# narayanan2004/GraphMat

Measured on AMD Instinct MI355X. Metric: GTEPS (edges/s) per iter + achieved HBM GB/s, PageRank RMAT-26, higher is better.
Workload: dtype f32

## Files before the change

### include/graphmat/kernels.hpp

```cpp
#pragma once
#include <hip/hip_runtime.h>
#include <stdint.h>
#include <string.h>

#include <type_traits>

#include "../graphmat_hip.h"

namespace GraphMat {

enum reduce_kind {
  REDUCE_AUTO = -1,
  REDUCE_ORDERED = 0,
  REDUCE_COMMUTATIVE = 1,
  REDUCE_LAST = 2,
  REDUCE_F32_ADD = 3
};

template <class P>
struct program_traits {
  static constexpr reduce_kind reduce = REDUCE_AUTO;
};

template <class P>
// ... 951 lines not shown
      const int v = stream_load(&A.colidx[k]);
      c[r] = pos < lr ? v : -1;
    }
  };
  auto msgs = [&]() {
#pragma unroll
    for (int r = 0; r < G; r++) {
      const int cc = c[r];
      const unsigned rel = (unsigned)(cc - hot.base);
      bool in_lds = rel < (unsigned)hot.nhot;
      unsigned slot = rel;
#ifdef GRAPHMAT_ABLATION
      if (cc >= 0 && abl_cold(cc, hot.cold_from, hot.base)) { in_lds = true; slot = (unsigned)cc & 4095u; }
      if (dbg & DBG_SKIP_GATHER) { in_lds = true; slot = 0; }
#endif
      const T mh = hot.s_hot[in_lds ? slot : 0u];
      const T* __restrict__ ga = (in_lds || cc < 0) ? xdummy : x + cc;
      const T mg = *ga;
      m[r] = in_lds ? mh : mg;
    }
  };
  cols(0);
  msgs();
  if (nsteps > 1) cols(1);
  for (int step = 0; step < nsteps; step++) {
#pragma unroll
    for (int r = 0; r < G; r++) {
      U term;
      const int kraw = __builtin_amdgcn_readlane(mt.e0, r) + step * 64 + lane;
      const int k = (int64_t)kraw < A.nnz ? kraw : (int)(A.nnz - 1);
      p.P::process_message(m[r], edge_at<E>(A.vals, k), no_vp, term);
      s_t[r][lane] = term;
    }
    __builtin_amdgcn_wave_barrier();
    if (step + 1 < nsteps) {
      msgs();
      if (step + 2 < nsteps) cols(step + 2);
    }
    if (lane < G && !(dbg & DBG_SKIP_FOLD)) {
      int n = mt.len - step * 64;
      n = n > 64 ? 64 : n;
      const U* t = s_t[lane];
      if (n == 64) {
        int k = 0;
        if (!has) { acc = t[0]; has = true; k = 1; }
        for (; k < 64; k++) { U v = t[k]; p.P::reduce_function(acc, v); }
      } else if (n > 0) {
        int k = 0;
        if (!has) { acc = t[0]; has = true; k = 1; }
        U nx[4];
        if (k + 4 <= n) {
#pragma unroll
          for (int u = 0; u < 4; u++) nx[u] = t[k + u];
        }
        while (k + 4 <= n) {
          U cur[4];
#pragma unroll
          for (int u = 0; u < 4; u++) cur[u] = nx[u];
          k += 4;
          if (k + 4 <= n) {
#pragma unroll
            for (int u = 0; u < 4; u++) nx[u] = t[k + u];
          }
#pragma unroll
          for (int u = 0; u < 4; u++) p.P::reduce_function(acc, cur[u]);
        }
        for (; k < n; k++) { U v = t[k]; p.P::reduce_function(acc, v); }
      }
    }
    __builtin_amdgcn_wave_barrier();
  }
  if (lane < G && mt.row >= 0 && has) {
    y[mt.row] = acc;
    if (!(accumulate & ACC_STATIC_BITS)) atomicOr(&ybits[mt.row >> 5], 1u << (mt.row & 31));
  }
}
template <class P, class T>
__device__ __forceinline__ bool w16_dense_ok(const gm_csr_t& A, const uint32_t* xbits, const uint32_t* want, const HotSet<T>& hot) {
  return xbits == nullptr && want == nullptr && !program_row_filter<P>::enabled && hot.NS == 1 && A.nnz < ((int64_t)1 << 31) && A.nnz > 0;
}

template <class P, class T, class U, class V, class E>
__global__ void __launch_bounds__(kWave16Block)
k_spmv_wave16(ProgArg<P> pa, gm_csr_t A, const int32_t* __restrict__ rows, int nlist, const T* __restrict__ x,
              const uint32_t* __restrict__ xbits, const V* __restrict__ vp, U* __restrict__ y,
              uint32_t* __restrict__ ybits, int accumulate GM_DBG_PARAM, const uint32_t* __restrict__ want) {
  static_assert(sizeof(U) == 4 || sizeof(U) == 8, "LDS tile of 4- or 8-byte products");
  constexpr int G = kWaveRows;
  constexpr int kStride = 64 + 16 / (int)sizeof(U);
  __shared__ __attribute__((aligned(16))) U s_t[kWave16Block / 64][G][kStride];
  __shared__ unsigned long long s_mask[kWave16Block / 64][G];
  constexpr int kHot = sizeof(T) == 4 ? kHotEntries : 1;
  __shared__ T s_hot[kHot];
  const HotSet<T> hot = hot_load<T, kHot, kWave16Block>(A, x, s_hot);
  __syncthreads();
  const P& p = *reinterpret_cast<const P*>(pa.b);
  const int wv = threadIdx.x >> 6, lane = threadIdx.x & 63;
  const int first = (blockIdx.x * (kWave16Block / 64) + wv) * G;
  if (first >= nlist) return;
  wave16_group<P, T, U, V, E, kStride>(p, A, rows, nlist, first, lane, x, xbits, vp, y, ybits, accumulate GM_DBG_PASS, want, hot, s_t[wv], s_mask[wv]);
}

template <class P, class T, class U, class V, class E, int BLOCK, int HOT>
__global__ void __launch_bounds__(BLOCK)
k_spmv_wave16p(ProgArg<P> pa, gm_csr_t A, const int32_t* __restrict__ rows, int nlist, const T* __restrict__ x,
               const uint32_t* __restrict__ xbits, const V* __restrict__ vp, U* __restrict__ y,
               uint32_t* __restrict__ ybits, int accumulate GM_DBG_PARAM, const uint32_t* __restrict__ want) {
  static_assert(sizeof(U) == 4 || sizeof(U) == 8, "LDS tile of 4- or 8-byte products");
  static_assert(sizeof(T) == 4, "4-byte messages");
  constexpr int G = kWaveRows;
  constexpr int kStride = 64 + 16 / (int)sizeof(U);
  __shared__ __attribute__((aligned(16))) U s_t[BLOCK / 64][G][kStride];
  __shared__ unsigned long long s_mask[BLOCK / 64][G];
  __shared__ T s_hot[HOT];
#ifdef GRAPHMAT_ABLATION
  const unsigned long long abl_t0 = wall_clock64();
#endif
  const HotSet<T> hot = hot_load<T, HOT, BLOCK>(A, x, s_hot);
  __syncthreads();
  const P& p = *reinterpret_cast<const P*>(pa.b);
  const int wv = threadIdx.x >> 6, lane = threadIdx.x & 63;
  const int ngroups = (nlist + G - 1) / G;
  const int nwaves = gridDim.x * (BLOCK / 64);
#ifdef GRAPHMAT_ABLATION
  const unsigned long long abl_t1 = wall_clock64();
  struct AblStamp {
    unsigned long long t0, t1;
    int w, lane;
    __device__ ~AblStamp() {
      if (lane == 0 && w < 8192) {
        g_abl_wave_times[0][w][0] = t0; g_abl_wave_times[0][w][1] = t1; g_abl_wave_times[0][w][2] = wall_clock64();
      }
    }
  } abl_stamp{abl_t0, abl_t1, (int)(blockIdx.x * (BLOCK / 64) + wv), lane};
#endif
  if (w16_dense_ok<P, T>(A, xbits, want, hot) && !(dbg & DBG_PLAIN_WAVE16)) {
    int g = wv * gridDim.x + blockIdx.x;
    int row_n = w16_row(rows, nlist, g + nwaves < ngroups ? (g + nwaves) * G : -1, lane);
    W16Meta<U> cur = w16_meta<U>(A, w16_row(rows, nlist, g < ngroups ? g * G : -1, lane), y, ybits, accumulate);
    while (g < ngroups) {
      const int gn = g + nwaves;
      const int row_nn = w16_row(rows, nlist, gn + nwaves < ngroups ? (gn + nwaves) * G : -1, lane);
      const W16Meta<U> nxt = w16_meta<U>(A, row_n, y, ybits, accumulate);
      wave16_dense<P, T, U, V, E, kStride>(p, A, cur, lane, x, y, ybits, accumulate GM_DBG_PASS, hot, s_t[wv]);
      cur = nxt;
      row_n = row_nn;
      g = gn;
    }
    return;
  }
  for (int g = wv * gridDim.x + blockIdx.x; g < ngroups; g += nwaves)
    wave16_group<P, T, U, V, E, kStride>(p, A, rows, nlist, g * G, lane, x, xbits, vp, y, ybits, accumulate GM_DBG_PASS, want, hot, s_t[wv], s_mask[wv]);
}

template <class P, class T, class U, class V, class E, int BLOCK, int HOT>
__global__ void __launch_bounds__(BLOCK)
k_spmv_rowwave(ProgArg<P> pa, gm_csr_t A, const T* __restrict__ x, U* __restrict__ y, uint32_t* __restrict__ ybits, int accumulate) {
  static_assert(sizeof(T) == 4, "4-byte messages");
  constexpr int W = BLOCK / 64;
  constexpr int CH = 512, PER = CH / 64;
  constexpr int kPadw = CH + CH / 32;
  __shared__ T s_hot[HOT > 0 ? HOT : 1];
  __shared__ T s_msg[W][kPadw];
#define GM_WSLOT(k) ((k) + ((k) >> 5))
#ifdef GRAPHMAT_ABLATION
  const unsigned long long abl_t0 = wall_clock64();
#endif
  const HotSet<T> hot = hot_load<T, HOT, BLOCK>(A, x, s_hot);
  __syncthreads();
  const P& p = *reinterpret_cast<const P*>(pa.b);
  const int wv = threadIdx.x >> 6, lane = threadIdx.x & 63;
#ifdef GRAPHMAT_ABLATION
  const unsigned long long abl_t1 = wall_clock64();
  struct AblStamp {
    unsigned long long t0, t1;
    int w, lane;
    __device__ ~AblStamp() {
      if (lane == 0 && w < 8192) {
        g_abl_wave_times[1][w][0] = t0; g_abl_wave_times[1][w][1] = t1; g_abl_wave_times[1][w][2] = wall_clock64();
      }
    }
  } abl_stamp{abl_t0, abl_t1, (int)(blockIdx.x * (BLOCK / 64) + wv), lane};
#endif
  T* sm = s_msg[wv];
  const int nwaves = gridDim.x * W;
  V no_vp;
  for (int b = wv * gridDim.x + blockIdx.x; b < A.nblk; b += nwaves) {
    const int sg = A.blk_seg[b];
    const int r0 = A.seg_row[sg], r1 = A.seg_row[sg + 1];
    for (int rg = r0; rg < r1; rg += 64) {
      const int row = rg + lane;
      int64_t rp0 = 0, rp1 = 0;
      if (row < r1) { rp0 = A.rowptr[row]; rp1 = A.rowptr[row + 1]; }
      const int lastl = (r1 - rg - 1) < 63 ? (r1 - rg - 1) : 63;
      const int64_t g0 = wave_bcast(rp0, 0), g1 = wave_bcast(rp1, lastl);
      bool has = false;
      U acc;
      if (rp1 > rp0 && (accumulate & ACC_READ_PREV) && bit_get(ybits, row)) { acc = y[row]; has = true; }
      for (int64_t c0 = g0; c0 < g1; c0 += CH) {
        const int n = (int)((g1 - c0) < CH ? (g1 - c0) : CH);
        int c[PER];
#pragma unroll
        for (int j = 0; j < PER; j++) {
          const int k = lane + 64 * j;
          c[j] = (k < n) ? stream_load(&A.colidx[c0 + k]) : -1;
        }
        T m[PER];
#pragma unroll
        for (int j = 0; j < PER; j++)
          if (c[j] >= 0) m[j] = hot.get(x, c[j]);
#pragma unroll
        for (int j = 0; j < PER; j++) {
          const int k = lane + 64 * j;
          if (k < n) sm[GM_WSLOT(k)] = m[j];
        }
        __builtin_amdgcn_wave_barrier();
        const int64_t ka = rp0 > c0 ? rp0 : c0, kb = rp1 < c0 + n ? rp1 : c0 + n;
        if (ka < kb) {
          int k = (int)(ka - c0);
          const int ke = (int)(kb - c0);
          if (!has) {
            p.P::process_message(sm[GM_WSLOT(k)], edge_at<E>(A.vals, c0 + k), no_vp, acc);
            has = true;
            k++;
          }
          for (; k + 4 <= ke; k += 4) {
            T r[4];
#pragma unroll
            for (int u = 0; u < 4; u++) r[u] = sm[GM_WSLOT(k + u)];
#pragma unroll
            for (int u = 0; u < 4; u++) {
              U res;
              p.P::process_message(r[u], edge_at<E>(A.vals, c0 + k + u), no_vp, res);
              p.P::reduce_function(acc, res);
            }
          }
          for (; k < ke; k++) {
            U res;
            p.P::process_message(sm[GM_WSLOT(k)], edge_at<E>(A.vals, c0 + k), no_vp, res);
            p.P::reduce_function(acc, res);
          }
        }
        __builtin_amdgcn_wave_barrier();
      }
      bool wrote = false;
      if (rp1 > rp0 && has) {
        y[row] = acc;
        wrote = true;
      }
      publish_row_bits(wrote, row, ybits, accumulate);
    }
  }
#undef GM_WSLOT
}

#ifdef GM_SELL_PHASE_TIMES
static __device__ unsigned long long g_sell_phase_ticks[4096][8];
#define GM_SELL_TICK(k) do { if constexpr (ABL & 8) { const unsigned long long t_ = wall_clock64(); if (lane == 0) g_sell_phase_ticks[wg * 16 + wv][k] += t_ - tphase; tphase = t_; } } while (0)
#else
#define GM_SELL_TICK(k) do { } while (0)
#endif
template <class P, class T, class U, class V, class E, bool HAS_VALS, int ABL, int UBATCH, int PIPE, int POOLW, bool SHARDED, int BLOCKT = 1024, bool SPARSE = false>
__device__ __forceinline__ void
sell_body(const ProgArg<P>& pa, int set, int stage_words, int nslices, int nrows_long, const int32_t* __restrict__ slice_base, const uint32_t* __restrict__ scol,
          const uint32_t* __restrict__ sval, const uint32_t* __restrict__ wrow, const int32_t* __restrict__ row_of_slot, const uint32_t* __restrict__ lcol,
          const uint32_t* __restrict__ lval, const uint32_t* __restrict__ lps, const int32_t* __restrict__ lrow_of_slot,
          const uint32_t* __restrict__ gcol, const uint32_t* __restrict__ gval, const uint32_t* __restrict__ gdst, const uint32_t* __restrict__ gslice,
          U* __restrict__ gterms , const T* __restrict__ x, U* __restrict__ y,
          int nsub, int stride, int hot_words, const uint32_t* __restrict__ xbits = nullptr, uint32_t* __restrict__ ybits = nullptr,
          U* __restrict__ sterms = nullptr ) {
  static_assert(sizeof(T) == 4 && sizeof(U) == 4, "4-byte messages and reductions");
  static_assert(!SPARSE || (PIPE == 2 && !SHARDED && ABL == 0), "the sparse form: single shard, two batches deep");
  constexpr int BLOCK = BLOCKT, W = BLOCK / 64, UB = UBATCH;
  constexpr int WS = 16;
  constexpr int ACC = GM_SWEEP_ACC_ROWS, NLP = GM_SWEEP_LONG_SLOTS;
  constexpr int KMAX = BLOCK == 1024 ? GM_SWEEP_MAX_STAGE / BLOCK : 12;
  static_assert(BLOCK >= NLP && BLOCK % 64 == 0, "the last GM_SWEEP_LONG_SLOTS threads fold the long rows");
  static_assert((POOLW + GM_SWEEP_ACC_ROWS) * 4 <= 160 * 1024, "k_spmv_sell: the pool and the accumulators must fit gfx950's 160 KB of LDS per workgroup");
  __shared__ uint32_t s_pool[POOLW];
  __shared__ uint32_t s_acc[ACC];
  __shared__ uint32_t s_hasbits[SPARSE ? (ACC + 31) / 32 : 1];
  __shared__ uint32_t s_stagebits[SPARSE ? GM_SWEEP_MAX_STAGE / 32 : 1];
  if constexpr (SPARSE) {
    for (int i = threadIdx.x; i < (ACC + 31) / 32; i += BLOCKT) s_hasbits[i] = 0u;
  }
  auto present = [&](uint32_t c4) { return ((xbits[c4 >> 7] >> ((c4 >> 2) & 31u)) & 1u) != 0u; };
  const P& p = *reinterpret_cast<const P*>(pa.b);
  const int wg = blockIdx.x, wv = __builtin_amdgcn_readfirstlane(threadIdx.x >> 6), lane = threadIdx.x & 63;
  const int HOT = POOLW - stage_words;
  uint32_t* const s_stage = s_pool + HOT;
  const char* __restrict__ xb = (const char*)x;
  V no_vp;
  const size_t vw = (size_t)set * 256 + wg;
  const int lj = (BLOCK - 1) - (int)threadIdx.x < NLP ? (BLOCK - 1) - (int)threadIdx.x : -1;
  bool lhas = false;
  U lacc;
  auto as_t = [](uint32_t raw) { T t; __builtin_memcpy(&t, &raw, 4); return t; };
  auto as_u = [](uint32_t raw) { U u; __builtin_memcpy(&u, &raw, 4); return u; };
  auto raw_u = [](const U& u) { uint32_t r; __builtin_memcpy(&r, &u, 4); return r; };
  auto as_e = [](uint32_t raw) { E e; if constexpr (HAS_VALS) __builtin_memcpy(&e, &raw, 4); else e = E(); return e; };
  constexpr int GK = 2;
  uint32_t pc[UB], pe[UB], lc[KMAX], le[KMAX], gc[GK], gd[GK], ge[GK];
  uint32_t pr = 0, prend = 0, pl0 = 0, pl1 = 0, pps = 0, ppe = 0, pga = 0, pgb = 0;
  auto prefetch = [&](int sl) {
    const size_t blk = vw * (size_t)nslices + (size_t)sl;
    const uint32_t* __restrict__ wr = wrow + blk * (WS + 1);
    pr = __builtin_amdgcn_readfirstlane(wr[wv]);
    prend = __builtin_amdgcn_readfirstlane(wr[wv + 1]);
#pragma unroll
    for (int j = 0; j < UB; j++) {
      const uint32_t rr = pr + j < prend ? pr + j : (prend > 0 ? prend - 1 : 0);
      pc[j] = __builtin_nontemporal_load(&scol[(size_t)rr * 64 + lane]);
      if constexpr (HAS_VALS) pe[j] = __builtin_nontemporal_load(&sval[(size_t)rr * 64 + lane]); else pe[j] = 0u;
    }
    if (gterms != nullptr) {
      const uint32_t g0 = gslice[sl], gn = gslice[sl + 1] - g0;
      pga = g0 + (uint32_t)((unsigned long long)gn * (unsigned)wg / 256ull);
      pgb = g0 + (uint32_t)((unsigned long long)gn * (unsigned)(wg + 1) / 256ull);
#pragma unroll
      for (int j = 0; j < GK; j++) {
        const uint32_t i = pga + (uint32_t)(j * BLOCK) + threadIdx.x;
        if (i < pgb) {
          gc[j] = __builtin_nontemporal_load(&gcol[i]);
          gd[j] = __builtin_nontemporal_load(&gdst[i]);
          if constexpr (HAS_VALS) ge[j] = __builtin_nontemporal_load(&gval[i]); else ge[j] = 0u;
        }
      }
    }
    if (nrows_long > 0 && !(ABL & 4)) {
      const size_t eb = blk * NLP;
      pl0 = lps[eb];
      pl1 = lps[eb + NLP];
      if (lj >= 0) { pps = lps[eb + lj]; ppe = lps[eb + lj + 1]; }
      const uint32_t n = pl1 - pl0 < (uint32_t)stage_words ? pl1 - pl0 : (uint32_t)stage_words;
#pragma unroll
      for (int j = 0; j < KMAX; j++) {
        if ((uint32_t)(j * BLOCK) < n) {
          const uint32_t i = (uint32_t)(j * BLOCK) + threadIdx.x;
          const uint32_t ii = pl0 + (i < n ? i : n - 1);
          lc[j] = __builtin_nontemporal_load(&lcol[ii]);
          if constexpr (HAS_VALS) le[j] = __builtin_nontemporal_load(&lval[ii]); else le[j] = 0u;
        }
      }
    }
  };
  prefetch(0);
  [[maybe_unused]] unsigned long long tphase = 0;
  if constexpr (ABL & 8) tphase = wall_clock64();
  for (int sl = 0; sl < nslices; sl++) {
    const int base = slice_base[sl];
    const int slen = slice_base[sl + 1] - base;
    int hq = 0;
    if constexpr (SHARDED) { const int cap = (hot_words < HOT ? hot_words : HOT) / nsub; hq = slen < cap ? slen : cap; }
    const int nhot = SHARDED ? hq * nsub : (slen < HOT ? slen : HOT);
    const uint32_t base4 = (uint32_t)base << 2, nhot4 = (uint32_t)nhot << 2;
    const uint32_t idle4 = SHARDED ? GM_SWEEP_HOT : base4;
    __syncthreads();
    GM_SELL_TICK(0);
    if constexpr (SHARDED) {
      for (int q = 0; q < nsub; q++) {
        const uint32_t* __restrict__ xq_ = (const uint32_t*)x + (size_t)q * (size_t)stride + (size_t)base;
        for (int i = threadIdx.x; i < hq; i += BLOCK) s_pool[q * hq + i] = xq_[i];
      }
    } else {
      for (int i = threadIdx.x; i < nhot; i += BLOCK) s_pool[i] = ((const uint32_t*)x)[base + i];
    }
    __syncthreads();
    GM_SELL_TICK(1);
    auto gather = [&](uint32_t c4) {
      if constexpr (SHARDED) {
        const bool h = (c4 & GM_SWEEP_HOT) != 0u;
        const uint32_t mh = *(const uint32_t*)((const char*)s_pool + (h ? (c4 & 0x3ffffffcu) : 0u));
        const uint32_t mg = *(const uint32_t*)(xb + (h ? base4 : c4));
        return h ? mh : mg;
      } else {
      const uint32_t rel4 = c4 - base4;
      if constexpr ((ABL & 3) == 1) return c4;
      if constexpr ((ABL & 3) == 2) return *(const uint32_t*)((const char*)s_pool + (nhot4 ? (rel4 % nhot4) & ~3u : 0u));
      const bool h = rel4 < nhot4;
      const uint32_t mh = *(const uint32_t*)((const char*)s_pool + (h ? rel4 : 0u));
      const uint32_t mg = *(const uint32_t*)(xb + (h ? base4 : c4));
      return h ? mh : mg;
      }
    };
    uint32_t gmsg[GK];
    const uint32_t ga = pga, gb = pgb;
    if (gterms != nullptr) {
#pragma unroll
      for (int j = 0; j < GK; j++)
        if (ga + (uint32_t)(j * BLOCK) + threadIdx.x < gb) gmsg[j] = gather(gc[j]);
    }
    if (nrows_long > 0 && !(ABL & 4)) {
      const uint32_t l0 = pl0, l1 = pl1, ps = pps, pe_ = ppe;
      for (uint32_t c0 = l0; c0 < l1; c0 += (uint32_t)stage_words) {
        const uint32_t n = l1 - c0 < (uint32_t)stage_words ? l1 - c0 : (uint32_t)stage_words;
        if (c0 != l0) {
          __syncthreads();
#pragma unroll
          for (int j = 0; j < KMAX; j++) {
            if ((uint32_t)(j * BLOCK) < n) {
              const uint32_t i = (uint32_t)(j * BLOCK) + threadIdx.x;
              const uint32_t ii = c0 + (i < n ? i : n - 1);
              lc[j] = __builtin_nontemporal_load(&lcol[ii]);
              if constexpr (HAS_VALS) le[j] = __builtin_nontemporal_load(&lval[ii]); else le[j] = 0u;
            }
          }
        }
        uint32_t m[KMAX];
#pragma unroll
        for (int j = 0; j < KMAX; j++)
          if ((uint32_t)(j * BLOCK) < n) {
            if constexpr (SPARSE) {
              const uint32_t i = (uint32_t)(j * BLOCK) + threadIdx.x;
              const bool pr = i < n && present(lc[j]);
              m[j] = gather(pr ? lc[j] : idle4);
              const unsigned long long pm = __ballot(pr);
              if (lane == 0) s_stagebits[(i >> 5)] = (uint32_t)pm;
              if (lane == 32) s_stagebits[(i >> 5)] = (uint32_t)(pm >> 32);
            } else {
              m[j] = gather(lc[j]);
            }
          }
#pragma unroll
        for (int j = 0; j < KMAX; j++) {
          const uint32_t i = (uint32_t)(j * BLOCK) + threadIdx.x;
          if (i < n) {
            U res;
            p.P::process_message(as_t(m[j]), as_e(le[j]), no_vp, res);
            s_stage[i] = raw_u(res);
          }
        }
        __syncthreads();
        GM_SELL_TICK(2);
        if (lj >= 0) {
          uint32_t k = ps > c0 ? ps : c0;
          const uint32_t ke = pe_ < c0 + n ? pe_ : c0 + n;
          if constexpr (SPARSE) {
            for (; k < ke; k++) {
              const uint32_t i = k - c0;
              if ((s_stagebits[i >> 5] >> (i & 31u)) & 1u) {
                if (lhas) p.P::reduce_function(lacc, as_u(s_stage[i])); else { lacc = as_u(s_stage[i]); lhas = true; }
              }
            }
          }
          if (k < ke && !lhas) { lacc = as_u(s_stage[k - c0]); lhas = true; k++; }
          for (; k + 4 <= ke; k += 4) {
            uint32_t r[4];
#pragma unroll
            for (int u = 0; u < 4; u++) r[u] = s_stage[k - c0 + u];
#pragma unroll
            for (int u = 0; u < 4; u++) p.P::reduce_function(lacc, as_u(r[u]));
          }
          for (; k < ke; k++) p.P::reduce_function(lacc, as_u(s_stage[k - c0]));
        }
      }
    }
    if (gterms != nullptr) {
#pragma unroll
      for (int j = 0; j < GK; j++) {
        if (ga + (uint32_t)(j * BLOCK) + threadIdx.x < gb) {
          U res;
          p.P::process_message(as_t(gmsg[j]), as_e(ge[j]), no_vp, res);
          gterms[gd[j]] = res;
        }
      }
      for (uint32_t i = ga + (uint32_t)(GK * BLOCK) + threadIdx.x; i < gb; i += BLOCK) {
        const uint32_t c = __builtin_nontemporal_load(&gcol[i]), d = __builtin_nontemporal_load(&gdst[i]);
        uint32_t e = 0u;
        if constexpr (HAS_VALS) e = __builtin_nontemporal_load(&gval[i]);
        U res;
        p.P::process_message(as_t(gather(c)), as_e(e), no_vp, res);
        gterms[d] = res;
      }
    }
    GM_SELL_TICK(3);
    uint32_t r = pr;
    const uint32_t rend = prend;
    uint32_t left = 0;
    int slot = 0x7fff;
    U acc;
    bool has = false;
    bool streaming = false;
    uint32_t srow = 0;
    if constexpr (PIPE == 2) {
      uint32_t cA[UB], eA[UB], mA[UB], cB[UB], eB[UB];
#pragma unroll
      for (int j = 0; j < UB; j++) { cA[j] = pc[j]; eA[j] = pe[j]; }
      auto load_entries = [&](uint32_t r0, uint32_t (&cx)[UB], uint32_t (&ex)[UB]) {
#pragma unroll
        for (int j = 0; j < UB; j++) {
          const uint32_t rr = r0 + j < rend ? r0 + j : rend - 1;
          cx[j] = __builtin_nontemporal_load(&scol[(size_t)rr * 64 + lane]);
          if constexpr (HAS_VALS) ex[j] = __builtin_nontemporal_load(&sval[(size_t)rr * 64 + lane]); else ex[j] = 0u;
        }
      };
      auto scan = [&](uint32_t r0, const uint32_t (&cx)[UB], uint32_t& skip) {
        uint32_t mask = 0;
        skip = 0;
#pragma unroll
        for (int j = 0; j < UB; j++) {
          if (r0 + j < rend) {
            if (left == 0) { mask |= 1u << j; left = ((uint32_t)__builtin_amdgcn_readfirstlane((int)cx[j]) >> 16) & 0x1fffu; }
            else left--;
          } else skip |= 1u << j;
        }
        skip |= mask;
        return mask;
      };
      auto gathers = [&](const uint32_t (&cx)[UB], uint32_t skip, uint32_t (&mx)[UB], uint32_t& px) {
        px = 0u;
#pragma unroll
        for (int j = 0; j < UB; j++) {
          if constexpr (SPARSE) {
            const bool real = !((skip >> j) & 1u) && (int32_t)cx[j] >= 0;
            const bool pr = real && present(cx[j]);
            px |= pr ? (1u << j) : 0u;
            mx[j] = gather(pr ? cx[j] : idle4);
          } else {
            mx[j] = gather(((skip >> j) & 1u) ? idle4 : (cx[j] & 0x7fffffffu));
          }
        }
      };
      if (r < rend) {
        uint32_t skipA = 0, maskA = scan(r, cA, skipA), pA = 0u;
        gathers(cA, skipA, mA, pA);
        load_entries(r + UB, cB, eB);
        while (true) {
          const uint32_t rn = r + UB;
          uint32_t mB[UB], cC[UB], eC[UB];
          uint32_t skipB = 0;
          const uint32_t maskB = scan(rn, cB, skipB);
          uint32_t pB = 0u;
          gathers(cB, skipB, mB, pB);
          load_entries(rn + UB, cC, eC);
#pragma unroll
          for (int j = 0; j < UB; j++) {
            if (r + j < rend) {
              if ((maskA >> j) & 1u) {
                if (slot != 0x7fff) {
                  s_acc[slot] = raw_u(acc);
                  if constexpr (SPARSE) { if (has) atomicOr(&s_hasbits[slot >> 5], 1u << (slot & 31)); }
                }
                slot = (int)(cA[j] & 0x7fffu);
                streaming = ((uint32_t)__builtin_amdgcn_readfirstlane((int)cA[j]) & 0x40000000u) != 0u;
                if (streaming) srow = (uint32_t)__ballot(((cA[j] >> 15) & 1u) != 0u);
                if constexpr (SPARSE) has = slot != 0x7fff && ((s_hasbits[slot >> 5] >> (slot & 31)) & 1u) != 0u;
                else has = !(cA[j] & 0x8000u);
                acc = as_u(slot != 0x7fff ? s_acc[slot] : 0u);
              } else if (streaming) {
                if (!SPARSE && sterms != nullptr && (int32_t)cA[j] >= 0) {
                  U res;
                  p.P::process_message(as_t(mA[j]), as_e(eA[j]), no_vp, res);
                  __builtin_nontemporal_store(raw_u(res), reinterpret_cast<uint32_t*>(sterms) + ((size_t)srow * 64 + lane));
                }
                srow++;
              } else if (SPARSE ? ((pA >> j) & 1u) != 0u : (int32_t)cA[j] >= 0) {
                U res;
                p.P::process_message(as_t(mA[j]), as_e(eA[j]), no_vp, res);
                if (has) p.P::reduce_function(acc, res);
                else acc = res;
                has = true;
              }
            }
          }
          r = rn;
          if (r >= rend) break;
          maskA = maskB;
          pA = pB;
#pragma unroll
          for (int j = 0; j < UB; j++) { cA[j] = cB[j]; eA[j] = eB[j]; mA[j] = mB[j]; cB[j] = cC[j]; eB[j] = eC[j]; }
        }
      }
    } else {
    uint32_t c[UB], ev[UB];
  #pragma unroll
      for (int j = 0; j < UB; j++) { c[j] = pc[j]; ev[j] = pe[j]; }
      auto entries = [&](uint32_t r0) {
  #pragma unroll
        for (int j = 0; j < UB; j++) {
          const uint32_t rr = r0 + j < rend ? r0 + j : rend - 1;
          c[j] = __builtin_nontemporal_load(&scol[(size_t)rr * 64 + lane]);
          if constexpr (HAS_VALS) ev[j] = __builtin_nontemporal_load(&sval[(size_t)rr * 64 + lane]); else ev[j] = 0u;
        }
      };
      while (r < rend) {
        uint32_t m[UB], cc[UB], e2[UB];
        uint32_t metamask = 0, l = left;
  #pragma unroll
        for (int j = 0; j < UB; j++) {
          if (r + j < rend) {
            if (l == 0) { metamask |= 1u << j; l = ((uint32_t)__builtin_amdgcn_readfirstlane((int)c[j]) >> 16) & 0x1fffu; }
            else l--;
          }
        }
  #pragma unroll
        for (int j = 0; j < UB; j++) {
          cc[j] = c[j];
          e2[j] = ev[j];
          m[j] = 0u;
          if (!((metamask >> j) & 1u)) m[j] = gather(c[j] & 0x7fffffffu);
        }
        const uint32_t r0 = r;
        r += UB;
        if (r < rend) entries(r);
  #pragma unroll
        for (int j = 0; j < UB; j++) {
          if (r0 + j < rend) {
            if ((metamask >> j) & 1u) {
              if (slot != 0x7fff) s_acc[slot] = raw_u(acc);
              slot = (int)(cc[j] & 0x7fffu);
              has = !(cc[j] & 0x8000u);
              acc = as_u(slot != 0x7fff ? s_acc[slot] : 0u);
            } else if ((int32_t)cc[j] >= 0) {
              U res;
              p.P::process_message(as_t(m[j]), as_e(e2[j]), no_vp, res);
              if (has) p.P::reduce_function(acc, res);
              else acc = res;
              has = true;
            }
          }
        }
        left = l;
      }
    }
    if (slot != 0x7fff) {
      s_acc[slot] = raw_u(acc);
      if constexpr (SPARSE) { if (has) atomicOr(&s_hasbits[slot >> 5], 1u << (slot & 31)); }
    }
    GM_SELL_TICK(4);
    if (sl + 1 < nslices) prefetch(sl + 1);
    GM_SELL_TICK(5);
  }
  __syncthreads();
  for (int i = threadIdx.x; i < ACC; i += BLOCK) {
    const int row = row_of_slot[vw * ACC + i];
    if constexpr (SPARSE) {
      if (row >= 0 && ((s_hasbits[i >> 5] >> (i & 31)) & 1u)) { y[row] = as_u(s_acc[i]); atomicOr(&ybits[row >> 5], 1u << (row & 31)); }
    } else {
      if (row >= 0) y[row] = as_u(s_acc[i]);
    }
  }
  if (lj >= 0 && nrows_long > 0) {
    const int row = lrow_of_slot[vw * NLP + lj];
    if (row >= 0 && lhas) {
      y[row] = lacc;
      if constexpr (SPARSE) atomicOr(&ybits[row >> 5], 1u << (row & 31));
    }
  }
}
template <class P, class T, class U, class V, class E, bool HAS_VALS, int ABL = 0, int UBATCH = 7, int PIPE = 2, int POOLW = GM_SWEEP_POOL>
__global__ void __launch_bounds__(1024)
k_spmv_sell(ProgArg<P> pa, int set, int stage_words, int nslices, int nrows_long, const int32_t* __restrict__ slice_base, const uint32_t* __restrict__ scol,
            const uint32_t* __restrict__ sval, const uint32_t* __restrict__ wrow, const int32_t* __restrict__ row_of_slot, const uint32_t* __restrict__ lcol,
            const uint32_t* __restrict__ lval, const uint32_t* __restrict__ lps, const int32_t* __restrict__ lrow_of_slot,
            const uint32_t* __restrict__ gcol, const uint32_t* __restrict__ gval, const uint32_t* __restrict__ gdst, const uint32_t* __restrict__ gslice,
            U* __restrict__ gterms, const T* __restrict__ x, U* __restrict__ y) {
  sell_body<P, T, U, V, E, HAS_VALS, ABL, UBATCH, PIPE, POOLW, false>(pa, set, stage_words, nslices, nrows_long, slice_base, scol, sval, wrow, row_of_slot, lcol, lval, lps,
                                                                       lrow_of_slot, gcol, gval, gdst, gslice, gterms, x, y, 1, 0, 0);
}
template <class P, class T, class U, class V, class E, bool HAS_VALS>
__global__ void __launch_bounds__(1024)
k_spmv_sell_stream(ProgArg<P> pa, int set, int stage_words, int nslices, int nrows_long, const int32_t* __restrict__ slice_base, const uint32_t* __restrict__ scol,
                   const uint32_t* __restrict__ sval, const uint32_t* __restrict__ wrow, const int32_t* __restrict__ row_of_slot, const uint32_t* __restrict__ lcol,
                   const uint32_t* __restrict__ lval, const uint32_t* __restrict__ lps, const int32_t* __restrict__ lrow_of_slot,
                   const uint32_t* __restrict__ gcol, const uint32_t* __restrict__ gval, const uint32_t* __restrict__ gdst, const uint32_t* __restrict__ gslice,
                   U* __restrict__ gterms, const T* __restrict__ x, U* __restrict__ y, U* __restrict__ sterms) {
  sell_body<P, T, U, V, E, HAS_VALS, 0, 7, 2, GM_SWEEP_POOL, false>(pa, set, stage_words, nslices, nrows_long, slice_base, scol, sval, wrow, row_of_slot, lcol, lval, lps,
                                                                     lrow_of_slot, gcol, gval, gdst, gslice, gterms, x, y, 1, 0, 0, nullptr, nullptr, sterms);
}
template <class P, class U>
__global__ void __launch_bounds__(512, 6)
k_short_fold(ProgArg<P> pa, const U* __restrict__ sterms, const uint16_t* __restrict__ sinv, const uint32_t* __restrict__ schunk, int nslices, int cap,
             const uint32_t* __restrict__ sbin_row, const uint32_t* __restrict__ soff, const int32_t* __restrict__ srow_id, U* __restrict__ y,
             uint32_t* __restrict__ ybits) {
  static_assert(sizeof(U) == 4, "4-byte reductions");
  __shared__ uint32_t s_prod[(GM_STREAM_BIN + 64) + (GM_STREAM_BIN + 64) / 32 + 1];
  auto at = [](uint32_t q) { return q + (q >> 5); };
  __shared__ uint32_t s_cpos[GM_MAX_SLICES], s_cpre[GM_MAX_SLICES + 1];
  const P& p = *reinterpret_cast<const P*>(pa.b);
  const int b = blockIdx.x, wv = threadIdx.x >> 6, lane = threadIdx.x & 63;
  const uint32_t* __restrict__ raw = reinterpret_cast<const uint32_t*>(sterms);
  const uint32_t i0 = sbin_row[b], i1 = sbin_row[b + 1], base = (uint32_t)b * (uint32_t)cap;
  constexpr int RK = 4;
  uint32_t ro0[RK], ro1[RK];
  int rid[RK];
#pragma unroll
  for (int j = 0; j < RK; j++) {
    const uint32_t i = i0 + (uint32_t)(j * 512) + threadIdx.x;
    if (i < i1) { ro0[j] = soff[i]; ro1[j] = soff[i + 1]; rid[j] = srow_id[i]; }
  }
  if ((int)threadIdx.x < nslices) {
    const uint2 pn = *reinterpret_cast<const uint2*>(&schunk[((size_t)b * nslices + threadIdx.x) * 2]);
    s_cpos[threadIdx.x] = pn.x;
    s_cpre[threadIdx.x] = pn.y;
  }
  __syncthreads();
  constexpr int CB = 4, CK = 4;
  for (int c0 = wv; c0 < nslices; c0 += 8 * CB) {
    uint32_t vv[CB][CK];
    uint16_t qq[CB][CK];
    uint32_t cp[CB], cn[CB];
#pragma unroll
    for (int c = 0; c < CB; c++) {
      const int sl = c0 + 8 * c;
      cp[c] = sl < nslices ? s_cpos[sl] : 0u;
      cn[c] = sl < nslices ? s_cpre[sl] : 0u;
    }
#pragma unroll
    for (int c = 0; c < CB; c++) {
#pragma unroll
      for (int k = 0; k < CK; k++) {
        const uint32_t i = (uint32_t)(k * 64 + lane);
        if (i < cn[c]) {
          vv[c][k] = __builtin_nontemporal_load(&raw[cp[c] + i]);
          qq[c][k] = __builtin_nontemporal_load(&sinv[cp[c] + i]);
        }
      }
    }
#pragma unroll
    for (int c = 0; c < CB; c++) {
#pragma unroll
      for (int k = 0; k < CK; k++)
        if ((uint32_t)(k * 64 + lane) < cn[c]) s_prod[at(qq[c][k])] = vv[c][k];
      for (uint32_t i = (uint32_t)(CK * 64 + lane); i < cn[c]; i += 64u) s_prod[at(sinv[cp[c] + i])] = raw[cp[c] + i];
    }
  }
  __syncthreads();
  auto as_u = [](uint32_t r) { U u; __builtin_memcpy(&u, &r, 4); return u; };
  for (uint32_t ii = i0 + (uint32_t)(wv * 64), jj = 0; ii < i1; ii += 512u, jj++) {
    const uint32_t i = ii + (uint32_t)lane;
    const bool valid = i < i1;
    int row = 0;
    if (valid) {
      uint32_t o0, o1;
      if (jj < RK) {
        o0 = ro0[0]; o1 = ro1[0]; row = rid[0];
#pragma unroll
        for (int j = 1; j < RK; j++) if ((int)jj == j) { o0 = ro0[j]; o1 = ro1[j]; row = rid[j]; }
      } else { o0 = soff[i]; o1 = soff[i + 1]; row = srow_id[i]; }
      o0 -= base; o1 -= base;
      U acc = as_u(s_prod[at(o0)]);
      for (uint32_t k = o0 + 1; k < o1; k++) p.P::reduce_function(acc, as_u(s_prod[at(k)]));
      y[row] = acc;
    }
    if (ybits != nullptr) {
      const int r0 = __builtin_amdgcn_readfirstlane(row);
      if (__all(!valid || row == r0 + lane)) {
        const unsigned long long hb = __ballot(valid);
        const int sh = r0 & 31;
        const unsigned long long lo = hb << sh, hi = sh ? (hb >> (64 - sh)) : 0ull;
        const uint32_t w = lane == 0 ? (uint32_t)lo : lane == 1 ? (uint32_t)(lo >> 32) : lane == 2 ? (uint32_t)hi : 0u;
        if (lane < 3 && w != 0u) atomicOr(&ybits[(r0 >> 5) + lane], w);
      } else if (valid) {
        atomicOr(&ybits[row >> 5], 1u << (row & 31));
      }
    }
  }
}
template <class P, class T, class U, class V, class E, bool HAS_VALS>
__global__ void __launch_bounds__(kBlock)
k_giant_gather_sliced(ProgArg<P> pa, const uint32_t* __restrict__ gcol, const uint32_t* __restrict__ gval, const uint32_t* __restrict__ gdst, int64_t n,
                      const T* __restrict__ x, U* __restrict__ gterms) {
  static_assert(sizeof(T) == 4 && sizeof(U) == 4, "4-byte messages and reductions");
  const P& p = *reinterpret_cast<const P*>(pa.b);
  V no_vp;
  for (int64_t i = (int64_t)blockIdx.x * kBlock + threadIdx.x; i < n; i += (int64_t)gridDim.x * kBlock) {
    const uint32_t c4 = __builtin_nontemporal_load(&gcol[i]), d = __builtin_nontemporal_load(&gdst[i]);
    E ev = E();
    if constexpr (HAS_VALS) { const uint32_t raw = __builtin_nontemporal_load(&gval[i]); __builtin_memcpy(&ev, &raw, 4); }
    const T m = *reinterpret_cast<const T*>(reinterpret_cast<const char*>(x) + c4);
    U res;
    p.P::process_message(m, ev, no_vp, res);
    gterms[d] = res;
  }
}

template <class P, class T, class U, class V, class E, bool HAS_VALS>
__global__ void __launch_bounds__(768)
k_spmv_sell_w12(ProgArg<P> pa, int set, int stage_words, int nslices, int nrows_long, const int32_t* __restrict__ slice_base, const uint32_t* __restrict__ scol,
                const uint32_t* __restrict__ sval, const uint32_t* __restrict__ wrow, const int32_t* __restrict__ row_of_slot, const uint32_t* __restrict__ lcol,
                const uint32_t* __restrict__ lval, const uint32_t* __restrict__ lps, const int32_t* __restrict__ lrow_of_slot,
                const uint32_t* __restrict__ gcol, const uint32_t* __restrict__ gval, const uint32_t* __restrict__ gdst, const uint32_t* __restrict__ gslice,
                U* __restrict__ gterms, const T* __restrict__ x, U* __restrict__ y) {
  sell_body<P, T, U, V, E, HAS_VALS, 0, 7, 2, GM_SWEEP_POOL_W12, false, 768>(pa, set, stage_words, nslices, nrows_long, slice_base, scol, sval, wrow, row_of_slot, lcol, lval, lps,
                                                                             lrow_of_slot, gcol, gval, gdst, gslice, gterms, x, y, 1, 0, 0);
}

template <class P, class T, class U, class V, class E, bool HAS_VALS>
__global__ void __launch_bounds__(1024)
k_spmv_sell_sparse(ProgArg<P> pa, int set, int stage_words, int nslices, int nrows_long, const int32_t* __restrict__ slice_base, const uint32_t* __restrict__ scol,
                   const uint32_t* __restrict__ sval, const uint32_t* __restrict__ wrow, const int32_t* __restrict__ row_of_slot, const uint32_t* __restrict__ lcol,
                   const uint32_t* __restrict__ lval, const uint32_t* __restrict__ lps, const int32_t* __restrict__ lrow_of_slot, const T* __restrict__ x,
                   const uint32_t* __restrict__ xbits, U* __restrict__ y, uint32_t* __restrict__ ybits) {
  sell_body<P, T, U, V, E, HAS_VALS, 0, 7, 2, GM_SWEEP_POOL_SPARSE, false, 1024, true>(pa, set, stage_words, nslices, nrows_long, slice_base, scol, sval, wrow, row_of_slot, lcol, lval,
                                                                                        lps, lrow_of_slot, nullptr, nullptr, nullptr, nullptr, (U*)nullptr, x, y, 1, 0, 0, xbits, ybits);
}

template <class P, class T, class U, class V, class E, bool HAS_VALS>
__global__ void __launch_bounds__(1024)
k_spmv_sell_sharded(ProgArg<P> pa, int set, int stage_words, int nslices, int nrows_long, const int32_t* __restrict__ slice_base, const uint32_t* __restrict__ scol,
                    const uint32_t* __restrict__ sval, const uint32_t* __restrict__ wrow, const int32_t* __restrict__ row_of_slot, const uint32_t* __restrict__ lcol,
                    const uint32_t* __restrict__ lval, const uint32_t* __restrict__ lps, const int32_t* __restrict__ lrow_of_slot,
                    const uint32_t* __restrict__ gcol, const uint32_t* __restrict__ gval, const uint32_t* __restrict__ gdst, const uint32_t* __restrict__ gslice,
                    U* __restrict__ gterms, const T* __restrict__ x, U* __restrict__ y, int nsub, int stride, int hot_words, U* __restrict__ sterms) {
  sell_body<P, T, U, V, E, HAS_VALS, 0, 7, 2, GM_SWEEP_POOL, true>(pa, set, stage_words, nslices, nrows_long, slice_base, scol, sval, wrow, row_of_slot, lcol, lval, lps,
                                                                    lrow_of_slot, gcol, gval, gdst, gslice, gterms, x, y, nsub, stride, hot_words, nullptr, nullptr, sterms);
}

template <class P, class T, class U, class V, class E, bool HAS_VALS, int UB = 2>
__global__ void __launch_bounds__(1024)
k_spmv_blocked(ProgArg<P> pa, const uint32_t* __restrict__ ecol, const uint16_t* __restrict__ erow, const uint32_t* __restrict__ eval, const uint32_t* __restrict__ woff, int nslices, int nblk,
               const int32_t* __restrict__ row_of, const T* __restrict__ x, U* __restrict__ y, unsigned int* __restrict__ step_count, int nsteps, int window) {
  static_assert(sizeof(T) == 4 && sizeof(U) == 4, "4-byte messages and reductions");
  extern __shared__ uint32_t s_bacc[];
  const P& p = *reinterpret_cast<const P*>(pa.b);
  const int lane = threadIdx.x & 63, wave = threadIdx.x >> 6;
  const unsigned int nwg = (gridDim.x + 7 - (blockIdx.x & 7)) >> 3;
  unsigned int* const mycnt = step_count + (size_t)(blockIdx.x & 7) * nsteps;
  const int npass = (nblk + (int)gridDim.x - 1) / (int)gridDim.x;
  V no_vp;
  bool gave_up = false;
  auto as_u = [](uint32_t raw) { U u; __builtin_memcpy(&u, &raw, 4); return u; };
  auto raw_u = [](const U& u) { uint32_t r; __builtin_memcpy(&r, &u, 4); return r; };
  auto as_e = [](uint32_t raw) { E e; if constexpr (HAS_VALS) __builtin_memcpy(&e, &raw, 4); else e = E(); return e; };
  for (int pass = 0; pass < npass; pass++) {
    const int blk = pass * (int)gridDim.x + (int)blockIdx.x;
    const bool has_blk = blk < nblk;
    uint32_t ws = 0, we = 0;
    if (has_blk) { const uint32_t* wo = woff + ((size_t)blk * nslices) * 17 + wave; ws = wo[0]; we = wo[1]; }
    uint32_t c[UB], r[UB], ev[UB];
    uint32_t pre = ws;
#pragma unroll
    for (int u = 0; u < UB; u++) { c[u] = ecol[pre + u * 64 + lane]; r[u] = erow[pre + u * 64 + lane]; if constexpr (HAS_VALS) ev[u] = eval[pre + u * 64 + lane]; else ev[u] = 0u; }
    for (int sl = 0; sl < nslices; sl++) {
      uint32_t nws = 0, nwe = 0;
      if (has_blk && sl + 1 < nslices) { const uint32_t* wo = woff + ((size_t)blk * nslices + sl + 1) * 17 + wave; nws = wo[0]; nwe = wo[1]; }
      if (pre != ws && ws < we) {
        pre = ws;
#pragma unroll
        for (int u = 0; u < UB; u++) { c[u] = ecol[pre + u * 64 + lane]; r[u] = erow[pre + u * 64 + lane]; if constexpr (HAS_VALS) ev[u] = eval[pre + u * 64 + lane]; else ev[u] = 0u; }
      }
      for (uint32_t p0 = ws; p0 < we;) {
        T m[UB];
#pragma unroll
        for (int u = 0; u < UB; u++) m[u] = x[c[u]];
        const uint32_t np0 = p0 + 64 * UB;
        const uint32_t nxt = np0 < we ? np0 : nws;
        uint32_t nc[UB], nr[UB], ne[UB];
#pragma unroll
        for (int u = 0; u < UB; u++) { nc[u] = ecol[nxt + u * 64 + lane]; nr[u] = erow[nxt + u * 64 + lane]; if constexpr (HAS_VALS) ne[u] = eval[nxt + u * 64 + lane]; else ne[u] = 0u; }
#pragma unroll
        for (int u = 0; u < UB; u++) {
          const bool valid = p0 + u * 64 + lane < we;
          const uint32_t id = valid ? (r[u] & 0x7fffu) : (0x10000u + lane);
          const uint32_t prev = __shfl_up(id, 1);
          const bool head = valid && (lane == 0 || id != prev);
          const unsigned long long H = __ballot(head) | __ballot(!valid);
          const unsigned long long above = lane == 63 ? 0ull : (H >> (lane + 1));
          const int runlen = above ? (__builtin_ctzll(above) + 1) : (64 - lane);
          U res;
          __builtin_memset(&res, 0, 4);
          if (valid) p.P::process_message(m[u], as_e(ev[u]), no_vp, res);
          const uint32_t rraw = raw_u(res);
          U acc = res;
          if (head && !(r[u] & 0x8000u)) { acc = as_u(s_bacc[id]); p.P::reduce_function(acc, res); }
          for (int k = 1; __ballot(head && k < runlen); k++) {
            const U t = as_u(__shfl(rraw, (lane + k) & 63));
            if (head && k < runlen) p.P::reduce_function(acc, t);
          }
          if (head) s_bacc[id] = raw_u(acc);
        }
#pragma unroll
        for (int u = 0; u < UB; u++) { c[u] = nc[u]; r[u] = nr[u]; ev[u] = ne[u]; }
        pre = nxt;
        p0 = np0;
      }
      __syncthreads();
      if (window > 0) {
        const int step = pass * nslices + sl;
        if (threadIdx.x == 0) {
          __hip_atomic_fetch_add(&mycnt[step], 1u, __ATOMIC_RELAXED, __HIP_MEMORY_SCOPE_AGENT);
          const int need = step + 1 - window;
          if (need >= 0 && !gave_up) {
            int tries = 0;
            for (; tries < 1000; tries++) {
              if (__hip_atomic_load(&mycnt[need], __ATOMIC_RELAXED, __HIP_MEMORY_SCOPE_AGENT) >= nwg) break;
              __builtin_amdgcn_s_sleep(4);
            }
            if (tries == 1000) gave_up = true;
          }
        }
        __syncthreads();
      }
      ws = nws; we = nwe;
    }
    if (has_blk) {
      const int32_t* __restrict__ ro = row_of + (size_t)blk * GM_BLOCKED_ROWS;
      for (int i = threadIdx.x; i < GM_BLOCKED_ROWS; i += 1024) {
        const int row = ro[i];
        if (row >= 0) y[row] = as_u(s_bacc[i]);
      }
    }
    __syncthreads();
  }
}

template <class P, class T, class U, class V, class E, bool USE_VP, int LPR>
__device__ __forceinline__ void group_rows_last(const P& p, const gm_csr_t& A, const int row, const int64_t e0, const int64_t e1,
                                                const unsigned long long todo, const int lane, const T* __restrict__ x,
                                                const uint32_t* __restrict__ xbits, const V* __restrict__ vp, U* __restrict__ y,
                                                uint32_t* __restrict__ ybits, const int accumulate,
                                                const uint32_t* __restrict__ xsum, unsigned char* s_idx ) {
  static_assert(LPR == 8 || LPR == 16 || LPR == 32, "lanes per row");
  const bool dense = (xbits == nullptr);
  const int nw = __popcll(todo);
  if ((todo >> lane) & 1ull) s_idx[__popcll(todo & ((1ull << lane) - 1ull))] = (unsigned char)lane;
  __builtin_amdgcn_wave_barrier();
  const int g = lane / LPR, sub = lane % LPR;
  const int e0l = (int)(uint32_t)e0, e0h = (int)(e0 >> 32), e1l = (int)(uint32_t)e1, e1h = (int)(e1 >> 32);
  int cur = 0, depth = 2, next = 0;
  int64_t lo = 0, hi = 0;
  bool active = false;
  constexpr int DMAX = 8;
  while (true) {
    const unsigned long long idle = __ballot(!active && sub == 0);
    const int k = next + __popcll(idle & ((1ull << (g * LPR)) - 1ull));
    const bool take = !active && k < nw;
    const int src = take ? (int)s_idx[k] : 0;
    const int r2 = __shfl(row, src, 64);
    const int a_l = __shfl(e0l, src, 64), a_h = __shfl(e0h, src, 64), b_l = __shfl(e1l, src, 64), b_h = __shfl(e1h, src, 64);
    if (take) {
      cur = r2;
      lo = ((int64_t)a_h << 32) | (uint32_t)a_l;
// ... 1407 lines not shown
```

Measured before the change: 327.8.

## Batch slice descriptors per lane, stage hot x via global_load_lds, split gathers

Per-slice descriptor words (row ranges, global-term bounds, long-row ranges, slice base) are now loaded in one vector load, one word per lane, then broadcast with readlane. This replaces several scalar dependent loads, and the loads for the next slice are issued before the barrier. The hot x window is copied into LDS with global_load_lds direct-to-LDS transfers instead of register round-trips. Gathers are split into separate cold (global) and hot (LDS) load phases so more loads are in flight, and the long-row staging is refactored into a lambda. This adds register pressure and relies on hand-written waitcnt values and an inline-asm pin, which are fragile.

```diff
diff --git a/include/graphmat/kernels.hpp b/include/graphmat/kernels.hpp
--- a/include/graphmat/kernels.hpp
+++ b/include/graphmat/kernels.hpp
@@ -1277,11 +1277,26 @@
   constexpr int GK = 2;
   uint32_t pc[UB], pe[UB], lc[KMAX], le[KMAX], gc[GK], gd[GK], ge[GK];
   uint32_t pr = 0, prend = 0, pl0 = 0, pl1 = 0, pps = 0, ppe = 0, pga = 0, pgb = 0;
-  auto prefetch = [&](int sl) {
+  const bool with_long = nrows_long > 0 && !(ABL & 4);
+  auto descriptors = [&](int sl) {
     const size_t blk = vw * (size_t)nslices + (size_t)sl;
-    const uint32_t* __restrict__ wr = wrow + blk * (WS + 1);
-    pr = __builtin_amdgcn_readfirstlane(wr[wv]);
-    prend = __builtin_amdgcn_readfirstlane(wr[wv + 1]);
+    const uint32_t* __restrict__ wr = wrow + blk * (WS + 1) + wv;
+    const uint32_t* __restrict__ gs = gterms != nullptr ? gslice + sl : (const uint32_t*)slice_base;
+    const uint32_t* __restrict__ lp = with_long ? lps + blk * NLP : (const uint32_t*)slice_base;
+    const uint32_t* q = (const uint32_t*)slice_base + sl + 1;
+    q = lane == 0 ? wr : q;
+    q = lane == 1 ? wr + 1 : q;
+    q = lane == 2 ? gs : q;
+    q = lane == 3 ? gs + 1 : q;
+    q = lane == 4 ? lp : q;
+    q = lane == 5 ? lp + (with_long ? NLP : 1) : q;
+    return *q;
+  };
+  auto desc_word = [](uint32_t dv, int k) { return (uint32_t)__builtin_amdgcn_readlane((int)dv, k); };
+  auto prefetch = [&](int sl, const uint32_t dv) {
+    const size_t blk = vw * (size_t)nslices + (size_t)sl;
+    pr = desc_word(dv, 0);
+    prend = desc_word(dv, 1);
 #pragma unroll
     for (int j = 0; j < UB; j++) {
       const uint32_t rr = pr + j < prend ? pr + j : (prend > 0 ? prend - 1 : 0);
@@ -1289,28 +1304,29 @@
       if constexpr (HAS_VALS) pe[j] = __builtin_nontemporal_load(&sval[(size_t)rr * 64 + lane]); else pe[j] = 0u;
     }
     if (gterms != nullptr) {
-      const uint32_t g0 = gslice[sl], gn = gslice[sl + 1] - g0;
+      const uint32_t g0 = desc_word(dv, 2), gn = desc_word(dv, 3) - g0;
       pga = g0 + (uint32_t)((unsigned long long)gn * (unsigned)wg / 256ull);
       pgb = g0 + (uint32_t)((unsigned long long)gn * (unsigned)(wg + 1) / 256ull);
 #pragma unroll
       for (int j = 0; j < GK; j++) {
         const uint32_t i = pga + (uint32_t)(j * BLOCK) + threadIdx.x;
+        gc[j] = 0u; gd[j] = 0u; ge[j] = 0u;
         if (i < pgb) {
           gc[j] = __builtin_nontemporal_load(&gcol[i]);
           gd[j] = __builtin_nontemporal_load(&gdst[i]);
-          if constexpr (HAS_VALS) ge[j] = __builtin_nontemporal_load(&gval[i]); else ge[j] = 0u;
-        }
-      }
-    }
-    if (nrows_long > 0 && !(ABL & 4)) {
+          if constexpr (HAS_VALS) ge[j] = __builtin_nontemporal_load(&gval[i]);
+        }
+      }
+    }
+    if (with_long) {
       const size_t eb = blk * NLP;
-      pl0 = lps[eb];
-      pl1 = lps[eb + NLP];
+      pl0 = desc_word(dv, 4);
+      pl1 = desc_word(dv, 5);
       if (lj >= 0) { pps = lps[eb + lj]; ppe = lps[eb + lj + 1]; }
       const uint32_t n = pl1 - pl0 < (uint32_t)stage_words ? pl1 - pl0 : (uint32_t)stage_words;
-#pragma unroll
-      for (int j = 0; j < KMAX; j++) {
-        if ((uint32_t)(j * BLOCK) < n) {
+      if (n > 0) {
+#pragma unroll
+        for (int j = 0; j < KMAX; j++) {
           const uint32_t i = (uint32_t)(j * BLOCK) + threadIdx.x;
           const uint32_t ii = pl0 + (i < n ? i : n - 1);
           lc[j] = __builtin_nontemporal_load(&lcol[ii]);
@@ -1319,12 +1335,14 @@
       }
     }
   };
-  prefetch(0);
+  auto pin = [](uint32_t& v) { asm volatile("" : "+v"(v)); };
+  uint32_t dn = descriptors(0);
+  prefetch(0, dn);
+  int base = slice_base[0], bnext = (int)desc_word(dn, 6);
   [[maybe_unused]] unsigned long long tphase = 0;
   if constexpr (ABL & 8) tphase = wall_clock64();
   for (int sl = 0; sl < nslices; sl++) {
-    const int base = slice_base[sl];
-    const int slen = slice_base[sl + 1] - base;
+    const int slen = bnext - base;
     int hq = 0;
     if constexpr (SHARDED) { const int cap = (hot_words < HOT ? hot_words : HOT) / nsub; hq = slen < cap ? slen : cap; }
     const int nhot = SHARDED ? hq * nsub : (slen < HOT ? slen : HOT);
@@ -1338,70 +1356,83 @@
         for (int i = threadIdx.x; i < hq; i += BLOCK) s_pool[q * hq + i] = xq_[i];
       }
     } else {
-      for (int i = threadIdx.x; i < nhot; i += BLOCK) s_pool[i] = ((const uint32_t*)x)[base + i];
-    }
+      typedef __attribute__((address_space(1))) const void* gptr_t;
+      typedef __attribute__((address_space(3))) void* lptr_t;
+      const uint32_t* __restrict__ xs = (const uint32_t*)x + base;
+      __builtin_amdgcn_s_waitcnt(0x0f70);
+#pragma nounroll
+      for (int k0 = 0; k0 < nhot; k0 += BLOCK) {
+        const int i = k0 + (int)threadIdx.x;
+        if (i < nhot) __builtin_amdgcn_global_load_lds((gptr_t)(xs + i), (lptr_t)(s_pool + k0 + wv * 64), 4, 0, 0);
+      }
+    }
+    dn = descriptors(sl + 1 < nslices ? sl + 1 : sl);
+    if constexpr (!SHARDED) __builtin_amdgcn_s_waitcnt(0);
     __syncthreads();
+    pin(dn);
     GM_SELL_TICK(1);
-    auto gather = [&](uint32_t c4) {
-      if constexpr (SHARDED) {
-        const bool h = (c4 & GM_SWEEP_HOT) != 0u;
-        const uint32_t mh = *(const uint32_t*)((const char*)s_pool + (h ? (c4 & 0x3ffffffcu) : 0u));
-        const uint32_t mg = *(const uint32_t*)(xb + (h ? base4 : c4));
-        return h ? mh : mg;
-      } else {
-      const uint32_t rel4 = c4 - base4;
-      if constexpr ((ABL & 3) == 1) return c4;
-      if constexpr ((ABL & 3) == 2) return *(const uint32_t*)((const char*)s_pool + (nhot4 ? (rel4 % nhot4) & ~3u : 0u));
-      const bool h = rel4 < nhot4;
-      const uint32_t mh = *(const uint32_t*)((const char*)s_pool + (h ? rel4 : 0u));
-      const uint32_t mg = *(const uint32_t*)(xb + (h ? base4 : c4));
-      return h ? mh : mg;
-      }
+    auto is_hot = [&](uint32_t c4) {
+      if constexpr (SHARDED) return (c4 & GM_SWEEP_HOT) != 0u;
+      else return c4 - base4 < nhot4;
     };
-    uint32_t gmsg[GK];
+    auto gather_cold = [&](uint32_t c4) {
+      if constexpr (!SHARDED && (ABL & 3) != 0) return c4;
+      else return *(const uint32_t*)(xb + (is_hot(c4) ? base4 : c4));
+    };
+    auto gather_hot = [&](uint32_t c4) {
+      if constexpr (SHARDED) return *(const uint32_t*)((const char*)s_pool + (is_hot(c4) ? (c4 & 0x3ffffffcu) : 0u));
+      else if constexpr ((ABL & 3) == 1) return c4;
+      else if constexpr ((ABL & 3) == 2) return *(const uint32_t*)((const char*)s_pool + (nhot4 ? ((c4 - base4) % nhot4) & ~3u : 0u));
+      else return *(const uint32_t*)((const char*)s_pool + (is_hot(c4) ? c4 - base4 : 0u));
+    };
+    auto gather_pick = [&](uint32_t c4, uint32_t mg, uint32_t mh) {
+      if constexpr (!SHARDED && (ABL & 3) != 0) return mh;
+      else return is_hot(c4) ? mh : mg;
+    };
+    auto gather = [&](uint32_t c4) { return gather_pick(c4, gather_cold(c4), gather_hot(c4)); };
+    uint32_t gsel[GK], gmg[GK], gmh[GK];
     const uint32_t ga = pga, gb = pgb;
     if (gterms != nullptr) {
 #pragma unroll
-      for (int j = 0; j < GK; j++)
-        if (ga + (uint32_t)(j * BLOCK) + threadIdx.x < gb) gmsg[j] = gather(gc[j]);
-    }
-    if (nrows_long > 0 && !(ABL & 4)) {
+      for (int j = 0; j < GK; j++) gsel[j] = ga + (uint32_t)(j * BLOCK) + threadIdx.x < gb ? gc[j] : idle4;
+#pragma unroll
+      for (int j = 0; j < GK; j++) gmg[j] = gather_cold(gsel[j]);
+#pragma unroll
+      for (int j = 0; j < GK; j++) gmh[j] = gather_hot(gsel[j]);
+    }
+    if (with_long) {
       const uint32_t l0 = pl0, l1 = pl1, ps = pps, pe_ = ppe;
-      for (uint32_t c0 = l0; c0 < l1; c0 += (uint32_t)stage_words) {
-        const uint32_t n = l1 - c0 < (uint32_t)stage_words ? l1 - c0 : (uint32_t)stage_words;
-        if (c0 != l0) {
-          __syncthreads();
-#pragma unroll
-          for (int j = 0; j < KMAX; j++) {
+      auto stage_round = [&](const uint32_t c0, const uint32_t n) {
+        uint32_t cs[KMAX], mg[KMAX], mh[KMAX];
+        [[maybe_unused]] uint32_t prm = 0u;
+#pragma unroll
+        for (int j = 0; j < KMAX; j++) {
+          const uint32_t i = (uint32_t)(j * BLOCK) + threadIdx.x;
+          bool live = i < n;
+          if constexpr (SPARSE) {
+            const bool there = present(lc[j]);
+            live = live & there;
+            prm |= live ? (1u << j) : 0u;
+          }
+          cs[j] = live ? lc[j] : idle4;
+        }
+#pragma unroll
+        for (int j = 0; j < KMAX; j++) mg[j] = gather_cold(cs[j]);
+#pragma unroll
+        for (int j = 0; j < KMAX; j++) mh[j] = gather_hot(cs[j]);
+#pragma unroll
+        for (int j = 0; j < KMAX; j++) {
+          const uint32_t i = (uint32_t)(j * BLOCK) + threadIdx.x;
+          if constexpr (SPARSE) {
             if ((uint32_t)(j * BLOCK) < n) {
-              const uint32_t i = (uint32_t)(j * BLOCK) + threadIdx.x;
-              const uint32_t ii = c0 + (i < n ? i : n - 1);
-              lc[j] = __builtin_nontemporal_load(&lcol[ii]);
-              if constexpr (HAS_VALS) le[j] = __builtin_nontemporal_load(&lval[ii]); else le[j] = 0u;
+              const unsigned long long pm = __ballot(((prm >> j) & 1u) != 0u);
+              if (lane == 0) s_stagebits[(i >> 5)] = (uint32_t)pm;
+              if (lane == 32) s_stagebits[(i >> 5)] = (uint32_t)(pm >> 32);
             }
           }
-        }
-        uint32_t m[KMAX];
-#pragma unroll
-        for (int j = 0; j < KMAX; j++)
-          if ((uint32_t)(j * BLOCK) < n) {
-            if constexpr (SPARSE) {
-              const uint32_t i = (uint32_t)(j * BLOCK) + threadIdx.x;
-              const bool pr = i < n && present(lc[j]);
-              m[j] = gather(pr ? lc[j] : idle4);
-              const unsigned long long pm = __ballot(pr);
-              if (lane == 0) s_stagebits[(i >> 5)] = (uint32_t)pm;
-              if (lane == 32) s_stagebits[(i >> 5)] = (uint32_t)(pm >> 32);
-            } else {
-              m[j] = gather(lc[j]);
-            }
-          }
-#pragma unroll
-        for (int j = 0; j < KMAX; j++) {
-          const uint32_t i = (uint32_t)(j * BLOCK) + threadIdx.x;
           if (i < n) {
             U res;
-            p.P::process_message(as_t(m[j]), as_e(le[j]), no_vp, res);
+            p.P::process_message(as_t(gather_pick(cs[j], mg[j], mh[j])), as_e(le[j]), no_vp, res);
             s_stage[i] = raw_u(res);
           }
         }
@@ -1428,6 +1459,19 @@
           }
           for (; k < ke; k++) p.P::reduce_function(lacc, as_u(s_stage[k - c0]));
         }
+      };
+      if (l0 < l1) stage_round(l0, l1 - l0 < (uint32_t)stage_words ? l1 - l0 : (uint32_t)stage_words);
+      for (uint32_t c0 = l0 + (uint32_t)stage_words; c0 < l1; c0 += (uint32_t)stage_words) {
+        const uint32_t n = l1 - c0 < (uint32_t)stage_words ? l1 - c0 : (uint32_t)stage_words;
+        __syncthreads();
+#pragma unroll
+        for (int j = 0; j < KMAX; j++) {
+          const uint32_t i = (uint32_t)(j * BLOCK) + threadIdx.x;
+          const uint32_t ii = c0 + (i < n ? i : n - 1);
+          lc[j] = __builtin_nontemporal_load(&lcol[ii]);
+          if constexpr (HAS_VALS) le[j] = __builtin_nontemporal_load(&lval[ii]); else le[j] = 0u;
+        }
+        stage_round(c0, n);
       }
     }
     if (gterms != nullptr) {
@@ -1435,7 +1479,7 @@
       for (int j = 0; j < GK; j++) {
         if (ga + (uint32_t)(j * BLOCK) + threadIdx.x < gb) {
           U res;
-          p.P::process_message(as_t(gmsg[j]), as_e(ge[j]), no_vp, res);
+          p.P::process_message(as_t(gather_pick(gsel[j], gmg[j], gmh[j])), as_e(ge[j]), no_vp, res);
           gterms[gd[j]] = res;
         }
       }
@@ -1603,7 +1647,9 @@
       if constexpr (SPARSE) { if (has) atomicOr(&s_hasbits[slot >> 5], 1u << (slot & 31)); }
     }
     GM_SELL_TICK(4);
-    if (sl + 1 < nslices) prefetch(sl + 1);
+    if (sl + 1 < nslices) prefetch(sl + 1, dn);
+    base = bnext;
+    bnext = (int)desc_word(dn, 6);
     GM_SELL_TICK(5);
   }
   __syncthreads();
```

After: 325.1. No clear change (-0.8%).
